# marcinjurek/pyMRA

Hardware: AMD Instinct MI355X
Metric: MRA nodes/sec, resident device pass (prior+posterior+likelihood+predict with tree and data in HBM; value_end_to_end = the same nodes over the wall-clock of MRATree(...)+getLikelihood()+predict()), 1024^2 grid M=6 J=4 r0=32 (higher is better)
Workload: dtype f64

## Files before the change

### pymra_amd/csrc/mra_kernels.h

```cpp
#pragma once
#include <hip/hip_runtime.h>
#include <stdint.h>

typedef double d4 __attribute__((ext_vector_type(4)));
typedef double d2 __attribute__((ext_vector_type(2)));
typedef int i4 __attribute__((ext_vector_type(4)));

#define MRA_AS1 __attribute__((address_space(1)))
__device__ __forceinline__ double gld(const double* p) { return *(const double MRA_AS1*)p; }
__device__ __forceinline__ int gldi(const int* p) { return *(const int MRA_AS1*)p; }
__device__ __forceinline__ d2 gld2(const double* p) { return *(const d2 MRA_AS1*)p; }
__device__ __forceinline__ d4 gld4(const double* p) { return *(const d4 MRA_AS1*)p; }
__device__ __forceinline__ void gst(double* p, double v) { *(double MRA_AS1*)p = v; }
__device__ __forceinline__ void gst2(double* p, d2 v) { *(d2 MRA_AS1*)p = v; }
__device__ __forceinline__ void gst4(double* p, d4 v) { *(d4 MRA_AS1*)p = v; }


#define MRA_YB 16
#ifdef MRA_WHATIF
#define MRA_WHATIF_BIT(dbg, bit) ((dbg) & (bit))
#else
#define MRA_WHATIF_BIT(dbg, bit) false
#endif
#define FT_LD 18
// ... 1841 lines not shown


#ifdef MRA_STAMPS
#define MRA_TSTAMP(slot) do { if (srow && (threadIdx.x & 63) == 0) srow[slot] = __builtin_amdgcn_s_memtime(); } while (0)
#define MRA_TSTAMP_ARG , unsigned long long* stamps
#define MRA_TSTAMP_ROW_ARG , unsigned long long* srow
#define MRA_TSTAMP_ROW(prob, t) , (stamps ? stamps + ((long)(prob) * 64 + (t)) * 8 : (unsigned long long*)nullptr)
#else
#define MRA_TSTAMP(slot) do { } while (0)
#define MRA_TSTAMP_ARG
#define MRA_TSTAMP_ROW_ARG
#define MRA_TSTAMP_ROW(prob, t)
#endif

__device__ __forceinline__ const double* trsm2_image_src(const Trsm2Prob& pb, int ntri, int e) {
    const int tile = e >> 7, chunk = e & 127, row = chunk >> 3, c2 = (chunk & 7) << 1;
    if (tile < ntri) {
        int jb = 1;
        while ((jb + 1) * jb / 2 <= tile) ++jb;
        const int kb = tile - jb * (jb - 1) / 2;
        return pb.L + (long)(jb * 16 + row) * pb.ldL + kb * 16 + c2;
    }
    return pb.invd + (long)(tile - ntri) * 256 + row * 16 + c2;
}

template <int I> struct Trsm2Step { static constexpr int value = I; };
template <int I, int N, class F>
__device__ __forceinline__ void trsm2_steps(int n, F f) {
    if constexpr (I < N) {
        if (I == 0 || I < n) { f(Trsm2Step<I>()); trsm2_steps<I + 1, N>(n, f); }
    }
}

template <int NTMAX, bool GATHER>
__device__ __forceinline__ void trsm2_row_tile(const Trsm2Prob& pb, const double* __restrict__ img, const int* __restrict__ sidx, int nt, int ntri,
                                               int t, int r, int q, int prow MRA_TSTAMP_ROW_ARG) {
    const d4 zero = {0, 0, 0, 0};
    MRA_TSTAMP(2);
    double* xp = pb.X + (long)t * 16 * pb.ldx + (long)r * pb.ldx + 4 * q;
    const double* lp = (pb.src && t >= pb.gtiles) ? pb.src + ((long)(t - pb.gtiles) * 16 + r) * pb.ldsrc + 4 * q : xp;
    d4 x[NTMAX];
    double ssq = 0.0;
    const bool with_var = pb.var && t >= pb.var_tile0;
    double* const vp = pb.var + (long)(t - pb.var_tile0) * 16 + r;
    if (nt <= 0) {
        if (with_var && q == 0) gst(vp, gld(vp) + pb.var_sign * ssq);
        return;
    }
    double var0 = 0.0;
    if (with_var && q == 0) var0 = gld(vp);
    if (GATHER) {
        const double* gp = pb.gW + t * 16 + r;
        trsm2_steps<0, NTMAX>(nt, [&](auto JB) __attribute__((always_inline)) {
            constexpr int jb = decltype(JB)::value;
            const i4 gi = *(const i4*)(sidx + jb * 16 + 4 * q);
#pragma unroll
            for (int j = 0; j < 4; ++j) x[jb][j] = gld(gp + (long)max(gi[j], 0) * pb.gld);
        });
    } else {
        trsm2_steps<0, NTMAX>(nt, [&](auto JB) __attribute__((always_inline)) { constexpr int jb = decltype(JB)::value; x[jb] = gld4(lp + jb * 16); });
    }
    if (GATHER) {
        trsm2_steps<0, NTMAX>(nt, [&](auto JB) __attribute__((always_inline)) {
            constexpr int jb = decltype(JB)::value;
            const i4 gi = *(const i4*)(sidx + jb * 16 + 4 * q);
#pragma unroll
            for (int j = 0; j < 4; ++j) x[jb][j] = gi[j] < 0 ? 0.0 : x[jb][j];
        });
    }
#ifdef MRA_STAMPS
    if (srow) { __builtin_amdgcn_s_waitcnt(0); MRA_TSTAMP(3); }
#endif
    trsm2_steps<0, NTMAX>(nt, [&](auto JB) __attribute__((always_inline)) {
        constexpr int jb = decltype(JB)::value;
        d4 acc = x[jb];
        d4 upd0 = zero, upd1 = zero;
#pragma unroll
        for (int kb = 0; kb < jb; ++kb) {
            const d4 a = *(const d4*)(img + (jb * (jb - 1) / 2 + kb) * 256 + prow * 16 + 4 * q);
            upd0 = mfma16(a[0], x[kb][0], upd0);
            upd1 = mfma16(a[1], x[kb][1], upd1);
            upd0 = mfma16(a[2], x[kb][2], upd0);
            upd1 = mfma16(a[3], x[kb][3], upd1);
        }
        if (jb > 0) acc -= upd0 + upd1;
        const d4 ia = *(const d4*)(img + (ntri + jb) * 256 + prow * 16 + 4 * q);
        d4 xx0 = mfma16(ia[0], acc[0], zero), xx1 = mfma16(ia[1], acc[1], zero);
        xx0 = mfma16(ia[2], acc[2], xx0);
        xx1 = mfma16(ia[3], acc[3], xx1);
        const d4 xx = xx0 + xx1;
        x[jb] = xx;
        gst4(xp + jb * 16, xx);
        ssq += xx[0] * xx[0] + xx[1] * xx[1] + xx[2] * xx[2] + xx[3] * xx[3];
    });
    MRA_TSTAMP(4);
    if (with_var) {
        ssq += __shfl_xor(ssq, 16, 64);
        ssq += __shfl_xor(ssq, 32, 64);
        if (q == 0) gst(vp, var0 + pb.var_sign * ssq);
    }
    MRA_TSTAMP(5);
}

template <int NTMAX>
__global__ __launch_bounds__(512) void k_trsm_rows2(const Trsm2Prob* __restrict__ probs, int tiles_per_wg MRA_TSTAMP_ARG) {
    extern __shared__ __attribute__((aligned(16))) double lds[];
    const Trsm2Prob pb = probs[blockIdx.y];
#ifdef MRA_STAMPS
    const unsigned long long t_wg0 = __builtin_amdgcn_s_memtime();
    const unsigned long long t_real0 = __builtin_amdgcn_s_memrealtime();
#endif
    const int t_begin = blockIdx.x * tiles_per_wg;
    if (t_begin >= pb.ntiles) return;
    const int t_end = min(pb.ntiles, t_begin + tiles_per_wg);
    const int nt = pb.nt;
    const int ntri = nt * (nt - 1) / 2;
    stage_chunks<8>(lds, (ntri + nt) * 128, [&](int e) -> const double* { return trsm2_image_src(pb, ntri, e); });
    int* const sidx = (int*)(lds + (long)(ntri + nt) * 256);
    if (pb.gtiles > 0 && t_begin < pb.gtiles)
        for (int e = threadIdx.x; e < nt * 16; e += blockDim.x) sidx[e] = gldi(pb.gidx + e);
    __syncthreads();
    const int wave = __builtin_amdgcn_readfirstlane(threadIdx.x >> 6), lane = threadIdx.x & 63, r = lane & 15, q = lane >> 4;
    const int nwave = blockDim.x >> 6;
    const int prow = pi16(r);
#ifdef MRA_STAMPS
    const unsigned long long t_wg1 = __builtin_amdgcn_s_memtime();
#endif
#ifdef MRA_STAMPS
#define MRA_T2_STAMP_HEAD(t) do { if (stamps && lane == 0) { stamps[((long)blockIdx.y * 64 + (t)) * 8 + 0] = t_wg0; stamps[((long)blockIdx.y * 64 + (t)) * 8 + 1] = t_wg1; } } while (0)
#define MRA_T2_STAMP_TAIL(t) do { if (stamps && lane == 0) { stamps[((long)blockIdx.y * 64 + (t)) * 8 + 6] = t_real0; stamps[((long)blockIdx.y * 64 + (t)) * 8 + 7] = __builtin_amdgcn_s_memrealtime(); } } while (0)
#else
#define MRA_T2_STAMP_HEAD(t) do { } while (0)
#define MRA_T2_STAMP_TAIL(t) do { } while (0)
#endif
    int t = t_begin + wave;
    for (; t < min(t_end, pb.gtiles); t += nwave) {
        MRA_T2_STAMP_HEAD(t);
        trsm2_row_tile<NTMAX, true>(pb, lds, sidx, nt, ntri, t, r, q, prow MRA_TSTAMP_ROW(blockIdx.y, t));
        MRA_T2_STAMP_TAIL(t);
    }
    for (; t < t_end; t += nwave) {
        MRA_T2_STAMP_HEAD(t);
        trsm2_row_tile<NTMAX, false>(pb, lds, sidx, nt, ntri, t, r, q, prow MRA_TSTAMP_ROW(blockIdx.y, t));
        MRA_T2_STAMP_TAIL(t);
    }
#undef MRA_T2_STAMP_HEAD
#undef MRA_T2_STAMP_TAIL
}

struct LeafSolveProb {
    const double* L;
    const double* invd;
    const double* V;
    const double* Ut;
    double* Wr;
    double* var;
    long ldL, ldx, ldw;
    int nt;
    int nrt;
    int nat;
    int zt;
};

#ifdef MRA_STAMPS
#define MRA_LSTAMP(slot) do { if (stamps && threadIdx.x == 0) stamps[(long)blockIdx.x * 8 + (slot)] = __builtin_amdgcn_s_memrealtime(); } while (0)
#define MRA_LSTAMP_ARG , unsigned long long* stamps
#else
#define MRA_LSTAMP(slot) do { } while (0)
#define MRA_LSTAMP_ARG
#endif
template <int NTMAX, int CT, bool LLDS>
__global__ __launch_bounds__(LLDS ? 512 : 256, LLDS ? 1 : 2) void k_leaf_solve_update(const LeafSolveProb* __restrict__ probs MRA_LSTAMP_ARG) {
    extern __shared__ __attribute__((aligned(16))) double lds[];
    MRA_LSTAMP(0);
    constexpr int NTHR = LLDS ? 512 : 256;
    constexpr int NWAVE = NTHR / 64;
    constexpr int NST = (CT * 64 + NTHR - 1) / NTHR;
    const LeafSolveProb* __restrict__ pp = probs + blockIdx.x;
    const int wave = __builtin_amdgcn_readfirstlane(threadIdx.x >> 6);
    const int lane = threadIdx.x & 63, r = lane & 15, q = lane >> 4;
// ... 2199 lines not shown
```

### pymra_amd/csrc/mra_plan.hip

```cpp
#include "mra_plan_types.h"
#include "mra_topology.h"
#include <atomic>
#include <chrono>
#include <memory>
#include <mutex>
#include <thread>

namespace {
struct PlanTrace {
    bool on;
    double t0, last;
    const char* what;
    static double now() { return std::chrono::duration<double, std::milli>(std::chrono::steady_clock::now().time_since_epoch()).count(); }
    explicit PlanTrace(const char* w) : on(getenv("MRA_TRACE_PLAN") != nullptr), t0(now()), last(t0), what(w) {}
    void mark(const char* label) { if (on) { const double t = now(); fprintf(stderr, "  [%s] %-34s %7.2f ms\n", what, label, t - last); last = t; } }
    ~PlanTrace() { if (on) fprintf(stderr, "  [%s] total %.2f ms (descriptor uploads of this thread so far: %ld, %.2f ms)\n", what, now() - t0, upload_stats().n, upload_stats().ms); }
};
}

#include <map>
#include <unordered_map>
namespace {
struct DevPool {
    std::mutex mu;
// ... 1099 lines not shown
    pl->gLeafSolve.upload(sp);
    pl->gLeafUpdatePlain.upload(in_order(d.upd, order));
    std::vector<LeafSolveProb> half;
    pl->hLeafSolveHalfPos.clear();
    for (size_t k = 0; k < n_small; ++k) {
        const LeafSolveProb& q = sp[k];
        const int h0 = (q.nrt + 1) / 2;
        for (int part = 0; part < 2; ++part) {
            LeafSolveProb h = q;
            const int t0 = part ? h0 : 0, t1 = part ? q.nrt : h0;
            if (t1 <= t0) continue;
            h.V = q.V + (size_t)t0 * 16 * q.ldx; h.Wr = q.Wr + (size_t)t0 * 16 * q.ldw; h.var = q.var + (size_t)t0 * 16; h.nrt = t1 - t0;
            half.push_back(h);
            pl->hLeafSolveHalfPos.push_back(k);
        }
    }
    pl->n_leaf_solve_half = half.size();
    pl->gLeafSolveHalf.upload(half);
    pl->hLeafSolve = sp; pl->hLeafSolveHalf = half;
    std::vector<long> lr0(nl);
    std::vector<unsigned char> lup(nl, 0);
    for (size_t t = 0; t < nl; ++t) lr0[t] = pl->row0[pl->leaf_nodes[t]];
    for (size_t k = 0; k < n_small; ++k) lup[order[k]] = 1;
    pl->leaf_row0_dev.upload(lr0); pl->leaf_upd_dev.upload(lup);
    const int nts = pl->trsm_small_nt;
    pl->leaf_solve_lds = (size_t)((nts * (nts - 1) / 2 + nts) * FT_SZ + 2 * nat_max * 16 * LG_LD) * sizeof(double);
    pl->leaf_solve_ok = n_small > 0 && nat_max <= 13 && nat_max > 0 && pl->leaf_solve_lds <= 160 * 1024 && pl->leaf_max_rows >= 128;
}

static void build_big_leaf_tiles(mra_plan* pl, const std::vector<size_t>& order, size_t n_small) {
    typedef mra_plan::PriorKeep K;
    if (pl->keep.dirty == K::Dirty::Oversized && !pl->stale.n_wg) pl->stale.swap(pl->big);
    pl->big.n_wg = pl->big.n_tiles = 0;
    if (!pl->regular || n_small >= order.size()) return;
    const size_t nl = pl->leaf_nodes.size();
    std::vector<long> first(nl + 1, 0);
    for (size_t t = 0; t < nl; ++t) first[t + 1] = first[t] + (pl->row1[pl->leaf_nodes[t]] - pl->row0[pl->leaf_nodes[t]]) / 16;
    const long per_wg = pl->cascade_stage_all ? 8 : pl->cascade_wpw;
    std::vector<long> wg0;
    std::vector<int> wgn;
    for (size_t k = n_small; k < order.size(); ++k) {
        const size_t t = order[k];
        for (long a = first[t]; a < first[t + 1]; a += per_wg) { wg0.push_back(a); wgn.push_back((int)std::min(per_wg, first[t + 1] - a)); }
        pl->big.n_tiles += first[t + 1] - first[t];
    }
    pl->big.n_wg = (long)wg0.size();
    pl->big.wg0.upload(wg0); pl->big.wgn.upload(wgn);
}

static void build_leaf(mra_plan* pl, const double* y) {
    PlanTrace tr("build_leaf");
    ArenaScope arena(&pl->arena);
    pl->cphantom_valid = false;
    pl->resid_lists = pl->resid_refused = false;
    pl->slv.valid = false; pl->slv.built = false;
    pl->cov.built = false;
    pl->sit.built = false;
    LeafDescs d;
    build_obs_lists(pl, y, d);
    tr.mark("observation lists");
    pl->panel.alloc(std::max<long>(pl->leaf_poff.back(), 1));
    pl->leafInv.alloc(std::max<long>(pl->leaf_ioff.back(), 1));
    tr.mark("panel allocation");
    build_leaf_descriptors(pl, d);
    tr.mark("leaf descriptors (host)");
    upload_leaf_ut_and_clear_panels(pl);
    tr.mark("panel memset");
    pl->hLeafSyrk = d.syrk;
    build_parent_products(pl, d);
    tr.mark("parent / grandparent descriptors");
    std::vector<size_t> order;
    const size_t n_small = order_small_first(pl, order);
    pl->n_chol_small = pl->n_trsm_small = n_small;
    upload_leaf_descriptors(pl, d, order);
    build_big_panels(pl, d);
    build_leaf_row_solves(pl, d, order, n_small);
    build_leaf_solve_lists(pl, d, order, n_small);
    build_big_leaf_tiles(pl, order, n_small);
    arena.finish();
    tr.mark("descriptor arena to the device");
// ... 23 lines not shown

template <int EPI>
static void launch_gemm(mra_plan* pl, const GemmProb* probs, size_t nprob, long maxM, long maxN, bool allow_lds = true, bool lower_tri = false) {
    mra_launch_gemm(pl, EPI, probs, nprob, maxM, maxN, allow_lds, lower_tri);
}
template <int EPI>
static void launch_leaf_gemm(mra_plan* pl, const GemmProb* probs, size_t nprob) { mra_launch_leaf_gemm(pl, EPI, probs, nprob); }

static void launch_panel(mra_plan* pl, const PanelProb* probs, size_t nprob, int accumulate = 0) {
    if (!nprob) return;
    hipLaunchKernelGGL(k_panel_chol, dim3((unsigned)nprob), dim3(256), 0, pl->stream, probs, pl->dnode.p, pl->errflag.p, accumulate);
}
void mra_panel_chol(mra_plan* pl, const PanelProb* probs, size_t nprob, double* dn, int* err) {
    hipLaunchKernelGGL(k_panel_chol, dim3((unsigned)nprob), dim3(256), 0, pl->stream, probs, dn, err, 0);
}
void mra_sample_draw(mra_plan* pl, const SampleZ& zs, long Kn, double* zc) {
    hipLaunchKernelGGL(k_sample_draw, dim3((unsigned)((Kn * 16 + 255) / 256)), dim3(256), 0, pl->stream, zs, Kn, zc);
}

#ifdef MRA_STAMPS
static unsigned long long* stamp_buffer(DevVec<double>& b, size_t n) {
    if (b.n < n) { b.alloc(n); HIP_TRY(mraMemset(b.p, 0, b.n * sizeof(double))); HIP_TRY(hipDeviceSynchronize()); }
    return (unsigned long long*)b.p;
}
#define MRA_TSTAMP_VAL , tst
#define MRA_LSTAMP_VAL , (unsigned long long*)pl->kstamps2.p
#define MRA_LSTAMP_NUL , (unsigned long long*)nullptr
#else
#define MRA_TSTAMP_VAL
#define MRA_LSTAMP_VAL
#define MRA_LSTAMP_NUL
#endif

static bool launch_trsm2(mra_plan* pl, const Trsm2Prob* probs, size_t nprob, int nt, long max_tiles, int tiles_per_wg) {
    if (!pl->prepare_only && (!nprob || max_tiles <= 0 || nt <= 0)) return true;
    if (nt > TRSM2_MAX_NT) return false;
    ensure_big_lds(pl, {(const void*)k_trsm_rows2<2>, (const void*)k_trsm_rows2<4>, (const void*)k_trsm_rows2<LEAF_SMALL_TILES>, (const void*)k_trsm_rows2<TRSM2_MAX_NT>});
    if (pl->prepare_only) return true;
    const size_t lds = (size_t)(nt * (nt - 1) / 2 + nt) * 2048 + (size_t)nt * 16 * sizeof(int);
    const unsigned gx = (unsigned)((max_tiles + tiles_per_wg - 1) / tiles_per_wg);
    const unsigned tb = 512;
#ifdef MRA_STAMPS
    unsigned long long* tst = (nprob >= 1024 && max_tiles <= 64) ? stamp_buffer(pl->tstamps, nprob * 64 * 8) : nullptr;
#endif
    for (size_t off = 0; off < nprob; off += 65535) {
        dim3 grid(gx, (unsigned)std::min<size_t>(65535, nprob - off));
        if (nt <= 2) hipLaunchKernelGGL((k_trsm_rows2<2>), grid, dim3(tb), lds, pl->stream, probs + off, tiles_per_wg MRA_TSTAMP_VAL);
        else if (nt <= 4) hipLaunchKernelGGL((k_trsm_rows2<4>), grid, dim3(tb), lds, pl->stream, probs + off, tiles_per_wg MRA_TSTAMP_VAL);
        else if (nt <= LEAF_SMALL_TILES) hipLaunchKernelGGL((k_trsm_rows2<LEAF_SMALL_TILES>), grid, dim3(tb), lds, pl->stream, probs + off, tiles_per_wg MRA_TSTAMP_VAL);
        else hipLaunchKernelGGL((k_trsm_rows2<TRSM2_MAX_NT>), grid, dim3(tb), lds, pl->stream, probs + off, tiles_per_wg MRA_TSTAMP_VAL);
    }
    return true;
}

static void launch_level_row_solve(mra_plan* pl, int m, const Trsm2Prob* probs2, const TrsmNode* nodes, double* var) {
    LevelData& lv = pl->lev[m];
    if (launch_trsm2(pl, probs2, lv.nodes.size(), lv.cwt, lv.max_tiles, 32)) return;
    ensure_tile_lists(pl, m);
    hipLaunchKernelGGL(k_trsm_rows, dim3((unsigned)((lv.ntiles + 3) / 4)), dim3(256), 0, pl->stream, nodes, lv.tile_node.p, lv.tile_row0.p,
                       lv.ntiles, pl->W.p, (long)pl->ldw, lv.c0, var);
}

static void launch_parent_front(mra_plan* pl, int nacc, size_t nprob, size_t lds, const FrontProb* probs, bool pair = false) {
    ensure_big_lds(pl, {(const void*)k_parent_front<2>, (const void*)k_parent_front<4>, (const void*)k_parent_front<8>, (const void*)k_parent_front<12>,
                        (const void*)k_parent_front_pair<17>, (const void*)k_parent_front_pair<23>});
    const dim3 grid((unsigned)nprob);
    if (pair) {
        if (nacc == 17) hipLaunchKernelGGL(k_parent_front_pair<17>, grid, dim3(256), lds, pl->stream, probs, pl->parentSegs.p, pl->dnode.p, pl->errflag.p);
        else hipLaunchKernelGGL(k_parent_front_pair<23>, grid, dim3(256), lds, pl->stream, probs, pl->parentSegs.p, pl->dnode.p, pl->errflag.p);
        return;
    }
    switch (nacc) {
        case 2: hipLaunchKernelGGL(k_parent_front<2>, grid, dim3(512), lds, pl->stream, probs, pl->parentSegs.p, pl->dnode.p, pl->errflag.p); break;
        case 4: hipLaunchKernelGGL(k_parent_front<4>, grid, dim3(512), lds, pl->stream, probs, pl->parentSegs.p, pl->dnode.p, pl->errflag.p); break;
        case 8: hipLaunchKernelGGL(k_parent_front<8>, grid, dim3(512), lds, pl->stream, probs, pl->parentSegs.p, pl->dnode.p, pl->errflag.p); break;
        default: hipLaunchKernelGGL(k_parent_front<12>, grid, dim3(512), lds, pl->stream, probs, pl->parentSegs.p, pl->dnode.p, pl->errflag.p); break;
    }
}

enum class LeafPart { All, Small, Rest };
// ... 197 lines not shown
    std::vector<PanelProb> ch = pl->hLeafCholSorted;
    std::vector<Trsm2Prob> ts = pl->hLeafTrsmFullPlainG;
    std::vector<LeafSolveProb> sp = pl->hLeafSolve, half = pl->hLeafSolveHalf;
    for (size_t k = 0; k < nl; ++k) {
        const size_t t = order[k];
        ch[k].src = C0(t); ch[k].obs = pl->obs_idx.p + pl->obs_off_host[t]; ch[k].n_obs = pl->leaf_nobs_host[t];
        ts[k].src = V0(t); ts[k].ldsrc = pl->leaf_nop[t];
        sp[k].V = V0(t);
    }
    for (size_t h = 0; h < half.size(); ++h) {
        const size_t k = pl->hLeafSolveHalfPos[h];
        half[h].V = sp[k].V + (half[h].V - pl->hLeafSolve[k].V);
    }
    pl->kLeafCholSorted.upload(ch); pl->kLeafTrsmFullPlainG.upload(ts);
    pl->kLeafSolve.upload(sp); pl->kLeafSolveHalf.upload(half);
    pl->resid_lists = true;
}

enum class PriorRows { RunAll, KeepAll, KeepRerunDirty };
struct PriorStep { bool run_knots = true; PriorRows rows = PriorRows::RunAll; };
static PriorStep prior_step_for(const mra_plan* pl, const PassRoute& r) {
    typedef mra_plan::PriorKeep K;
    PriorStep s;
    const K& k = pl->keep;
    if (r.path != PassPath::Fused || pl->host_cov || !pl->use_prior_reuse || (pl->dbg & 7) || !k.knots_valid) return s;
    s.run_knots = false;
    if (r.scatter_ut) return s;
    const bool have = (k.rows == K::Rows::All && k.var_valid) || (r.lik_rows && k.rows == K::Rows::Observed && k.dirty == K::Dirty::Clean);
    if (!have || k.dirty == K::Dirty::All) return s;
    s.rows = k.dirty == K::Dirty::Clean ? PriorRows::KeepAll : PriorRows::KeepRerunDirty;
    return s;
}

static CascadeArgs prior_cascade_base(const mra_plan* pl) {
    CascadeArgs base{};
    base.ycol = -1;
    for (int m = 0; m < pl->NL; ++m) {
        base.lev[m].kx = pl->fl[m].kx.p; base.lev[m].kvalid = pl->fl[m].kvalid.p; base.lev[m].Wk = pl->fl[m].Wk.p;
        base.lev[m].L = pl->lev[m].Lp.p; base.lev[m].invd = pl->lev[m].invP.p;
        base.coff[m] = pl->coff[m];
    }
    base.X = pl->X.p; base.W = pl->W.p; base.ldw = pl->ldw;
    return base;
}

static void run_prior_fused_knots(mra_plan* pl, const CascadeArgs& base) {
    const int n_chain = pl->route.n_chain;
    if (n_chain) {
        Work fl;
        for (int m = 0; m < n_chain; ++m) fl += pl->lev[m].fl_pchol;
        KTimer kt(pl, KF_PRIOR_CHOL, fl);
        KnotChainArgs ka{};
        for (int m = 0; m < n_chain; ++m) {
            ka.lev[m] = base.lev[m];
            ka.node_base[m] = (int)pl->level_ptr[m];
        }
        ka.chain = pl->kc_chain.p; ka.ownmask = pl->kc_ownmask.p; ka.knots = pl->kc_knots.p; ka.nl = n_chain; ka.err = pl->errflag.p;
#ifdef MRA_STAMPS
        ka.stamps = stamp_buffer(pl->kstamps, pl->lev[n_chain - 1].nodes.size() * 64);
#endif
        launch_knot_chain(pl, ka);
    }
    for (int m = n_chain; m < pl->NL; ++m) {
        LevelData& lv = pl->lev[m];
        KTimer kt(pl, KF_PRIOR_CHOL, lv.fl_pchol);
        CascadeArgs ar = base;
// ... 17 lines not shown
        fl.alg *= share; fl.exec *= share; fl.bytes = share * 8.0 * pl->P * (pl->d + 1 + pl->ldw + 1);
    }
    else if (r.lik_rows) {
        ensure_lik_tiles(pl);
        const double share = 16.0 * (double)pl->n_lik_tiles / (double)std::max<long>(pl->P, 1);
        fl.alg *= share; fl.exec *= share; fl.bytes = share * 8.0 * pl->P * (pl->d + 1 + pl->ldw) + pl->by_leaf_ut;
    }
    KTimer kt(pl, KF_PRIOR_TRSM, fl);
    CascadeArgs ar = base;
    ar.knot_mode = 0; ar.mlast = pl->NL - 1; ar.dbg = pl->dbg;
#ifdef MRA_STAMPS
    ar.stamps = stamp_buffer(pl->stamps, (size_t)pl->n_ftiles * 16);
#endif
    ar.var_out = pl->var.p; ar.cov0 = kernel_cov0(pl);
    ar.ycol = pl->Ka; ar.y = pl->y.p;
    if (r.scatter_ut) {
        ar.obs_pos = pl->obs_pos.p; ar.tile_leaf = pl->ft_leaf.p; ar.leaf_ut = pl->leaf_ut.p; ar.leaf_nop = pl->leaf_nop_dev.p;
        ar.y = pl->y.p;
        for (int m = 0; m < pl->NL; ++m) ar.ut_off[m] = pl->coff[m] - pl->asuf[pl->NL];
        ar.ut_yrow = pl->Ka - pl->asuf[pl->NL];
    }
    if (pl->cascade_stage_all) { ar.n_wg = pl->n_fwg_leaf; ar.wg_tile0 = pl->ft_wg0_leaf.p; ar.wg_ntiles = pl->ft_wgn_leaf.p; }
    else { ar.n_wg = pl->n_fwg; ar.wg_tile0 = pl->ft_wg0.p; ar.wg_ntiles = pl->ft_wgn.p; }
    ar.tile_row0 = pl->ft_row0.p; ar.tile_chain = pl->ft_chain.p;
    if (r.lik_rows) ar.var_out = nullptr;
    if (only) { ar.n_wg = only->n_wg; ar.wg_tile0 = only->wg0.p; ar.wg_ntiles = only->wgn.p; }
    else if (r.lik_rows) {
        ar.row_gather = pl->obs_idx.p; ar.tile_chain = pl->lik_chain.p; ar.tile_leaf = pl->lik_leaf.p;
        ar.n_wg = pl->n_lik_wg; ar.wg_tile0 = pl->lik_wg0.p; ar.wg_ntiles = pl->lik_wgn.p;
    }
    launch_cascade_any(pl, ar);
}

static void run_prior_refresh(mra_plan* pl, bool with_var) {
    KTimer kt(pl, KF_MISC, Work(0.0, 0.0, 8.0 * 16.0 * pl->n_ftiles * (MRA_YB + (with_var ? 3 : 1))));
    const long n = pl->n_ftiles * 64;
    if (n <= 0) return;
    hipLaunchKernelGGL(k_refresh_yblock, dim3((unsigned)((n + 255) / 256)), dim3(256), 0, pl->stream, pl->W.p, (long)pl->ldw, pl->Ka, pl->y.p,
                       pl->ft_row0.p, pl->n_ftiles, with_var ? pl->var.p : (double*)nullptr, pl->var_prior.p);
}

static void keep_prior_var(mra_plan* pl) {
    if (pl->var_prior.n != (size_t)pl->P) pl->var_prior.alloc((size_t)pl->P);
    KTimer kt(pl, KF_MISC, Work(0.0, 0.0, 16.0 * pl->P));
    HIP_TRY(hipMemcpyAsync(pl->var_prior.p, pl->var.p, (size_t)pl->P * sizeof(double), hipMemcpyDeviceToDevice, pl->stream));
}

static void run_prior_fused(mra_plan* pl) {
    typedef mra_plan::PriorKeep K;
    const PassRoute& r = pl->route;
    const PriorStep step = prior_step_for(pl, r);
    const CascadeArgs base = prior_cascade_base(pl);
    K& k = pl->keep;
    if (step.run_knots) {
        prior_keep_reset(pl);
        run_prior_fused_knots(pl, base);
        k.knots_valid = true;
    }
    switch (step.rows) {
        case PriorRows::RunAll:
            run_prior_fused_rows(pl, base);
            k.rows = r.lik_rows ? K::Rows::Observed : K::Rows::All;
            k.dirty = K::Dirty::Clean;
            pl->stale.n_wg = pl->stale.n_tiles = 0;
            if (!r.lik_rows && pl->use_prior_reuse) { keep_prior_var(pl); k.var_valid = true; }
            return;
        case PriorRows::KeepRerunDirty:
            run_prior_refresh(pl, !r.lik_rows);
            run_prior_fused_rows(pl, base, pl->stale.n_wg ? &pl->stale : &pl->big);
            k.dirty = K::Dirty::Clean;
            pl->stale.n_wg = pl->stale.n_tiles = 0;
            return;
        case PriorRows::KeepAll:
            run_prior_refresh(pl, !r.lik_rows);
            return;
    }
}

static void run_predict_hi(mra_plan* pl) {
    const int NL = pl->NL, nlo = NL - 4;
    PredHiArgs hi{};
    Work fl_hi, fl_lo;
    for (int h = 0; h < 4; ++h) {
        const int m = nlo + h;
        hi.hi[h].F = pl->lev[m].F.p; hi.hi[h].invF = pl->lev[m].invF.p; hi.hi[h].nf = pl->lev[m].nf;
        hi.hi[h].ld = pl->lev[m].ldf; hi.hi[h].stride = (long)pl->lev[m].nf * pl->lev[m].ldf;
        hi.coff_hi[h] = pl->coff[m];
        fl_hi += pl->lev[m].fl_trsm + pl->lev[m].fl_update;
    }
    hi.W = pl->W.p; hi.var = pl->var.p; hi.ldw = pl->ldw;
    hi.col_low = pl->coff[nlo - 1]; hi.n_low = nlo * 4 + 1; hi.lev0 = nlo;
    hi.tile_row0 = pl->ft_row0.p; hi.tile_chain = pl->ft_chain.p; hi.wg_tile0 = pl->ft_wg0.p; hi.wg_ntiles = pl->ft_wgn.p;
    fl_hi.bytes = 8.0 * pl->P * (pl->ldw + (pl->ldw - pl->coff[nlo - 1]) + 2);
    const bool fold = pl->route.update == LeafUpdate::InPredictHi;
    if (fold) {
        hi.wg_leaf = pl->hi_wgleaf.p; hi.leaf_ut = pl->leaf_ut.p; hi.leaf_nop = pl->leaf_nop_dev.p; hi.leaf_row0 = pl->leaf_row0_dev.p; hi.na = pl->na[NL];
        fl_hi += Work(pl->fl_leaf_update.alg, pl->fl_leaf_update.exec, pl->by_leaf_tt + pl->by_leaf_ut);
    }
    PredArgs lo{};
    for (int m = 0; m < nlo; ++m) {
        lo.lev[m].F = pl->lev[m].F.p; lo.lev[m].invF = pl->lev[m].invF.p; lo.lev[m].nf = pl->lev[m].nf;
        lo.lev[m].ld = pl->lev[m].ldf; lo.lev[m].stride = (long)pl->lev[m].nf * pl->lev[m].ldf;
        lo.coff[m] = pl->coff[m];
        fl_lo += pl->lev[m].fl_trsm + pl->lev[m].fl_update;
    }
    lo.deep = lo.lev[nlo - 1];
    lo.W = pl->W.p; lo.mean = pl->mean.p; lo.var = pl->var.p; lo.ldw = pl->ldw; lo.ycol = pl->Ka;
    lo.tile_row0 = pl->ft_row0.p; lo.tile_chain = pl->ft_chain.p; lo.wg_tile0 = pl->hi_wg0_8.p; lo.wg_ntiles = pl->hi_wgn_8.p;
// ... 33 lines not shown
    if (ar.n_wg <= 0) return;
    launch_predict_any(pl, ar, lds);
}

static void phase_mark(mra_plan* pl, int k) { if (k == 0 || k == 5 || pl->ktiming) hipEventRecord(pl->ev[k], pl->stream); }

static void ensure_gt(mra_plan* pl) {
    if (pl->Gt.p || pl->leaf_goff.back() == 0) return;
    pl->Gt.alloc(pl->leaf_goff.back());
    for (size_t k = 0; k < pl->hKids.size(); ++k)
        if (pl->kid_leaf[k] >= 0) pl->hKids[k].G = pl->Gt.p + pl->leaf_goff[pl->kid_leaf[k]];
    pl->asmKids.upload(pl->hKids);
    for (size_t t = 0; t < pl->hLeafSyrk.size(); ++t) pl->hLeafSyrk[t].C = pl->Gt.p + pl->leaf_goff[t];
    pl->gLeafSyrk.upload(pl->hLeafSyrk);
}

static const PassRoute& open_pass(mra_plan* pl, uint32_t flags, bool full_rows) {
    if (g_dry) refuse_dry_run();
    if (!(pl->have_locs && pl->have_obs && pl->have_kernel))
        throw MraError(MRA_ERR_STATE, "mra_run needs set_locs, set_obs and set_kernel first");
    HIP_TRY(mraSetDevice(pl->device));
    if (pl->pass_open) {
        pl->cphantom_valid = false;
        prior_keep_reset(pl);
        if (pl->side_pending) HIP_TRY(hipStreamWaitEvent(pl->stream, pl->ev_join, 0));
        HIP_TRY(hipStreamSynchronize(pl->stream));
        HIP_TRY(hipStreamSynchronize(pl->stream2));
        HIP_TRY(hipMemsetAsync(pl->errflag.p, 0, sizeof(int), pl->stream));
        for (auto& e : pl->kev) { hipEventDestroy(e.second.first); hipEventDestroy(e.second.second); }
        pl->kev.clear();
    }
    pl->side_pending = false;
    pl->split_pending = false;
    pl->pass_open = true;
    pl->run_flags = flags;
    pl->slv.valid = false;
    for (int k = 0; k < KF_COUNT; ++k) pl->kstat[k] = mra_plan::KStat();
    if (!pl->lik_general_valid && route_for(pl, flags, full_rows).lik_general) ensure_lik_general(pl);
    pl->route = route_for(pl, flags, full_rows);
    pl->route_set = true;
    const PassRoute& r = pl->route;
    pl->leaf_fork = pl->use_leaf_fork && r.path == PassPath::Fused && r.chol == LeafChol::TilesSplit &&
                    0 < pl->n_trsm_small && pl->n_trsm_small < pl->leaf_nodes.size();
    return pl->route;
}

static void run_init_yblock(mra_plan* pl, const PassRoute& r) {
    KTimer kt(pl, KF_MISC, 0);
    const long n = pl->P * MRA_YB;
    hipLaunchKernelGGL(k_init_yblock, dim3((unsigned)((n + 255) / 256)), dim3(256), 0, pl->stream, pl->W.p,
                       (long)pl->ldw, pl->Ka, pl->y.p, pl->P, r.acc_var ? pl->var.p : (double*)nullptr, pl->host_cov ? 0.0 : kernel_cov0(pl),
                       pl->host_cov ? pl->covdiag.p : (const double*)nullptr);
}

static void run_prior_level_one_launch(mra_plan* pl, const PassRoute& r, LevelData& lv) {
    const size_t nn = lv.nodes.size();
    { KTimer kt(pl, KF_PRIOR_CHOL, lv.fl_knot_resid); launch_gemm<EPI_COV>(pl, lv.gKnotResid.p, nn, lv.cw, lv.cw); }
    { KTimer kt(pl, KF_PRIOR_CHOL, lv.fl_pchol); launch_panel(pl, lv.gPriorChol.p, nn); }
    if (r.lik_general) {
        Work w = lv.fl_resid + lv.fl_trsm.with_bytes(0.0);
        w.alg *= lv.lik_share; w.exec *= lv.lik_share; w.bytes *= lv.lik_share;
        KTimer kt(pl, KF_PRIOR_RESID, w);
        mra_launch_prior_level(pl, lv.gResidLik.p, lv.gResidLik.n);
    } else {
        KTimer kt(pl, KF_PRIOR_RESID, lv.fl_resid + lv.fl_trsm.with_bytes(0.0));
        mra_launch_prior_level(pl, lv.gResidFused.p, lv.gResidFused.n);
// ... 70 lines not shown
static void run_leaf_noise(mra_plan* pl, const PassRoute& r, size_t nl) {
    if (!pl->noise_on || resid_out_of_place(pl, r)) return;
    KTimer kt(pl, KF_MISC, 0);
    hipLaunchKernelGGL(k_leaf_noise, dim3((unsigned)((nl + 3) / 4)), dim3(256), 0, pl->stream, pl->gLeaf.p, pl->leaf_nobs.p, pl->noise.p, (int)nl);
}

struct SideFork {
    mra_plan* pl; hipStream_t main_stream; bool side; hipEvent_t joined;
    SideFork(mra_plan* p, bool on, hipEvent_t after, hipEvent_t joined_) : pl(p), main_stream(p->stream), side(on), joined(joined_) {
        if (!side) return;
        if (after) {
            HIP_TRY(hipEventRecord(after, main_stream));
            HIP_TRY(hipStreamWaitEvent(pl->stream2, after, 0));
        }
        pl->stream = pl->stream2;
    }
    void join() {
        if (!side) return;
        pl->stream = main_stream;
        HIP_TRY(hipEventRecord(joined, pl->stream2));
    }
    ~SideFork() { pl->stream = main_stream; }
};

static void run_leaf_chol_and_solve(mra_plan* pl, const PassRoute& r, size_t nl) {
    const int obs_tiles = pl->leaf_max_nop / 16;
    const int row_tiles = r.predict ? pl->leaf_max_tiles_full : pl->leaf_max_tiles_lik;
    if (r.path != PassPath::Fused) { launch_leaf_chol(pl, r, nl); launch_trsm2(pl, r.trsm_all, nl, obs_tiles, row_tiles, row_tiles); return; }
    const size_t n_small = pl->n_trsm_small;
    const int small_row_tiles = (r.predict && !r.solve_fused) ? pl->trsm_small_tiles_full : pl->trsm_small_tiles_lik;
    const bool oop = resid_out_of_place(pl, r);
    auto kept = [&](const Trsm2Prob* p) { return (oop && p == pl->gLeafTrsmFullPlainG.p) ? pl->kLeafTrsmFullPlainG.p : p; };
    const Trsm2Prob *trsm_all = kept(r.trsm_all), *trsm_small = kept(r.trsm_small);
    auto solve_rest = [&] { launch_trsm2(pl, trsm_all + n_small, nl - n_small, obs_tiles, row_tiles, (nl - n_small) < 512 ? 4 : row_tiles); };
    if (pl->leaf_fork) {
        SideFork fork(pl, true, pl->ev_leaf_fork, pl->ev_leaf_join);
        launch_leaf_chol(pl, r, nl, LeafPart::Rest);
        solve_rest();
        fork.join();
    }
    launch_leaf_chol(pl, r, nl, pl->leaf_fork ? LeafPart::Small : LeafPart::All);
    if (n_small) launch_trsm2(pl, trsm_small, n_small, pl->trsm_small_nt, small_row_tiles, small_row_tiles);
    if (pl->leaf_fork) HIP_TRY(hipStreamWaitEvent(pl->stream, pl->ev_leaf_join, 0));
    else if (nl > n_small) solve_rest();
}

static void run_leaf_big_panels(mra_plan* pl, const PassRoute& r, size_t nl) {
    const int v = r.predict ? 0 : 1;
    for (size_t st = 0; st < pl->gBigPanel[v].size(); ++st) {
        launch_panel(pl, pl->gBigPanel[v][st].p, nl, st > 0 ? 1 : 0);
        if (pl->bigM[v][st] > 0 && pl->bigN[v][st] > 0)
            launch_gemm<EPI_SUB>(pl, pl->gBigTrail[v][st].p, nl, pl->bigM[v][st], pl->bigN[v][st]);
    }
}

static void run_leaf_factor(mra_plan* pl, const PassRoute& r, size_t nl) {
    KTimer kt(pl, KF_LEAF_CHOL, r.predict ? pl->fl_leaf_chol : pl->fl_leaf_chol_lik);
    if (r.chol != LeafChol::BigPanels) run_leaf_chol_and_solve(pl, r, nl);
    else run_leaf_big_panels(pl, r, nl);
}

static void run_leaf_syrk(mra_plan* pl, size_t nl) {
    ensure_gt(pl);
    KTimer kt(pl, KF_LEAF_SYRK, pl->fl_leaf_syrk);
    launch_gemm<EPI_SET>(pl, pl->gLeafSyrk.p, nl, pl->leaf_max_na, pl->leaf_max_na, false, true);
}

static void run_leaf_var(mra_plan* pl, const PassRoute& r) {
    if (r.var == LeafVar::None) return;
    KTimer kt(pl, KF_MISC, 0);
    ensure_row_leaf(pl);
    if (r.var == LeafVar::FinishVar)
        hipLaunchKernelGGL(k_leaf_finish_var, dim3((unsigned)((pl->P + 255) / 256)), dim3(256), 0, pl->stream, pl->row_leaf.p, pl->W.p,
                           (long)pl->ldw, pl->Ka, pl->var.p, pl->P);
    else
// ... 1666 lines not shown
```

### pymra_amd/csrc/mra_plan_types.h

```cpp
#pragma once
#include "mra_kernels.h"
#include "../../include/mra_hip.h"

#include <algorithm>
#include <cmath>
#include <cstdio>
#include <cstdlib>
#include <cstring>
#include <dlfcn.h>
#include <functional>
#include <initializer_list>
#include <rccl/rccl.h>
#include <set>
#include <string>
#include <thread>
#include <vector>
#include <time.h>

#define MRA_VERSION_STR "mra_hip 0.2 (gfx950)"

static const bool g_dry = []() { const char* e = getenv("MRA_HOST_DRYRUN"); return e && e[0] == '1'; }();
hipError_t mraMalloc(void** p, size_t n);
hipError_t mraFree(void* p);
static inline hipError_t mraMemcpy(void* d, const void* s_, size_t n, hipMemcpyKind k) { if (g_dry) { memcpy(d, s_, n); return hipSuccess; } return hipMemcpy(d, s_, n, k); }
// ... 351 lines not shown
    struct PriorKeep {
        enum class Rows { None, Observed, All };
        enum class Dirty { Clean, Oversized, All };
        bool knots_valid = false;
        Rows rows = Rows::None;
        bool var_valid = false;
        Dirty dirty = Dirty::Clean;
    } keep;
    struct ResidKeep {
        enum class Form { None, COnly, Full };
        Form resid = Form::None;
        bool phantom = false;
    } rkeep;
    bool use_resid_reuse = true;
    DevVec<double> resid;
    std::vector<long> leaf_koff;
    bool resid_lists = false, resid_refused = false;
    std::vector<int> obs_list_host;
    std::vector<PanelProb> hLeafCholSorted;
    std::vector<Trsm2Prob> hLeafTrsmFullPlainG;
    std::vector<LeafSolveProb> hLeafSolve, hLeafSolveHalf;
    std::vector<size_t> hLeafSolveHalfPos;
    std::vector<LeafProb> hLeaf;
    DevVec<GemmProb> kLeafResid, kLeafResidLik;
    DevVec<PanelProb> kLeafCholSorted;
    DevVec<Trsm2Prob> kLeafTrsmFullPlainG;
    DevVec<LeafSolveProb> kLeafSolve, kLeafSolveHalf;
    DevVec<LeafProb> kLeaf;
    bool use_prior_reuse = true;
    DevVec<double> var_prior;
    struct LeafTileWgs {
        DevVec<long> wg0;
        DevVec<int> wgn;
        long n_wg = 0, n_tiles = 0;
        void swap(LeafTileWgs& o) { wg0.swap(o.wg0); wgn.swap(o.wgn); std::swap(n_wg, o.n_wg); std::swap(n_tiles, o.n_tiles); }
    } big, stale;
    int use_hi_fold = 1;
    bool use_prior_level = true;
    bool parent_panel_lds_ok = false;
    bool grand_syrk_dma_ok = false;
    bool grand_syrk_blk_ok = false;
    int use_syrk_blk = 1;
    bool seg_gemm_lds = true;
    bool use_pred_update = true;
    DevVec<long> leaf_row0_dev;
    DevVec<unsigned char> leaf_upd_dev;
    size_t leaf_solve_lds = 0;
    int leaf_solve_mode = 2;
    size_t n_trsm_small = 0;
    int trsm_small_nt = 0, trsm_small_tiles_full = 0, trsm_small_tiles_lik = 0;
    DevVec<GemmProb> gParentSyrk;
    DevVec<GemmSeg> parentSegs;
    DevVec<FrontProb> gParentFront;
    int parent_front_nacc = 0;
    size_t parent_front_lds = 0;
    int parent_pair_nacc = 0;
    size_t parent_pair_lds = 0;
    double parent_pair_idle_exec = 0;
    int use_parent_pair = 1;
    bool parent_syrk = false;
    bool lowrank_parent = false;
    DevVec<GemmProb> gParentPanel, gGrandSyrk;
    DevVec<GemmSeg> grandSegs, parentSegsAo;
    DevVec<FrontProb> gParentOwn;
    DevVec<Trsm2Prob> gParentZt;
    size_t parent_own_lds = 0;
    Work fl_parent_panel, fl_grand_syrk;
    bool shape_regular = false;
    std::vector<AsmChild> hKids;
// ... 337 lines not shown
```

Before: 1.719 million.

## Skip full prior refresh on kept passes by gathering y in leaf TRSM

On kept-prior passes the full-tile y-block and variance refresh is replaced by targeted work. The leaf triangular solve now gathers observations directly from y for the last gathered tile, zeroing missing or non-finite values. It reads the prior variance through an offset into the saved copy instead of restoring it. Only the big-leaf and empty-leaf tiles get a y-block refresh, and that refresh can run on the forked side stream. This removes a full-grid memory pass per predict call, at the cost of more control-flow state and more kernel instantiations.

```diff
diff --git a/pymra_amd/csrc/mra_kernels.h b/pymra_amd/csrc/mra_kernels.h
--- a/pymra_amd/csrc/mra_kernels.h
+++ b/pymra_amd/csrc/mra_kernels.h
@@ -1897,9 +1897,11 @@
     }
 }
 
-template <int NTMAX, bool GATHER>
+enum { TRSM2_STREAM = 0, TRSM2_GATHER = 1, TRSM2_YTILE = 2 };
+template <int NTMAX, int SRC>
 __device__ __forceinline__ void trsm2_row_tile(const Trsm2Prob& pb, const double* __restrict__ img, const int* __restrict__ sidx, int nt, int ntri,
-                                               int t, int r, int q, int prow MRA_TSTAMP_ROW_ARG) {
+                                               int t, int r, int q, int prow, const double* __restrict__ gy, long var_rd_off MRA_TSTAMP_ROW_ARG) {
+    constexpr bool GATHER = SRC == TRSM2_GATHER;
     const d4 zero = {0, 0, 0, 0};
     MRA_TSTAMP(2);
     double* xp = pb.X + (long)t * 16 * pb.ldx + (long)r * pb.ldx + 4 * q;
@@ -1909,11 +1911,11 @@
     const bool with_var = pb.var && t >= pb.var_tile0;
     double* const vp = pb.var + (long)(t - pb.var_tile0) * 16 + r;
     if (nt <= 0) {
-        if (with_var && q == 0) gst(vp, gld(vp) + pb.var_sign * ssq);
+        if (with_var && q == 0) gst(vp, gld(vp + var_rd_off) + pb.var_sign * ssq);
         return;
     }
     double var0 = 0.0;
-    if (with_var && q == 0) var0 = gld(vp);
+    if (with_var && q == 0) var0 = gld(vp + var_rd_off);
     if (GATHER) {
         const double* gp = pb.gW + t * 16 + r;
         trsm2_steps<0, NTMAX>(nt, [&](auto JB) __attribute__((always_inline)) {
@@ -1921,6 +1923,23 @@
             const i4 gi = *(const i4*)(sidx + jb * 16 + 4 * q);
 #pragma unroll
             for (int j = 0; j < 4; ++j) x[jb][j] = gld(gp + (long)max(gi[j], 0) * pb.gld);
+        });
+    } else if (SRC == TRSM2_YTILE) {
+        if (r == 0) {
+            trsm2_steps<0, NTMAX>(nt, [&](auto JB) __attribute__((always_inline)) {
+                constexpr int jb = decltype(JB)::value;
+                const i4 gi = *(const i4*)(sidx + jb * 16 + 4 * q);
+#pragma unroll
+                for (int j = 0; j < 4; ++j) x[jb][j] = gld(gy + max(gi[j], 0));
+            });
+        } else {
+            trsm2_steps<0, NTMAX>(nt, [&](auto JB) __attribute__((always_inline)) { constexpr int jb = decltype(JB)::value; x[jb] = zero; });
+        }
+        trsm2_steps<0, NTMAX>(nt, [&](auto JB) __attribute__((always_inline)) {
+            constexpr int jb = decltype(JB)::value;
+            const i4 gi = *(const i4*)(sidx + jb * 16 + 4 * q);
+#pragma unroll
+            for (int j = 0; j < 4; ++j) x[jb][j] = (gi[j] < 0 || !isfinite(x[jb][j])) ? 0.0 : x[jb][j];
         });
     } else {
         trsm2_steps<0, NTMAX>(nt, [&](auto JB) __attribute__((always_inline)) { constexpr int jb = decltype(JB)::value; x[jb] = gld4(lp + jb * 16); });
@@ -1967,8 +1986,8 @@
     MRA_TSTAMP(5);
 }
 
-template <int NTMAX>
-__global__ __launch_bounds__(512) void k_trsm_rows2(const Trsm2Prob* __restrict__ probs, int tiles_per_wg MRA_TSTAMP_ARG) {
+template <int NTMAX, bool LEAF>
+__device__ __forceinline__ void trsm2_rows(const Trsm2Prob* __restrict__ probs, int tiles_per_wg, const double* __restrict__ gy, long var_rd_off MRA_TSTAMP_ARG) {
     extern __shared__ __attribute__((aligned(16))) double lds[];
     const Trsm2Prob pb = probs[blockIdx.y];
 #ifdef MRA_STAMPS
@@ -1999,18 +2018,38 @@
 #define MRA_T2_STAMP_TAIL(t) do { } while (0)
 #endif
     int t = t_begin + wave;
-    for (; t < min(t_end, pb.gtiles); t += nwave) {
+    for (; t < min(t_end, pb.gtiles - (LEAF ? 1 : 0)); t += nwave) {
         MRA_T2_STAMP_HEAD(t);
-        trsm2_row_tile<NTMAX, true>(pb, lds, sidx, nt, ntri, t, r, q, prow MRA_TSTAMP_ROW(blockIdx.y, t));
+        trsm2_row_tile<NTMAX, TRSM2_GATHER>(pb, lds, sidx, nt, ntri, t, r, q, prow, gy, var_rd_off MRA_TSTAMP_ROW(blockIdx.y, t));
         MRA_T2_STAMP_TAIL(t);
+    }
+    if constexpr (LEAF) {
+        for (; t < min(t_end, pb.gtiles); t += nwave) {
+            MRA_T2_STAMP_HEAD(t);
+            trsm2_row_tile<NTMAX, TRSM2_YTILE>(pb, lds, sidx, nt, ntri, t, r, q, prow, gy, var_rd_off MRA_TSTAMP_ROW(blockIdx.y, t));
+            MRA_T2_STAMP_TAIL(t);
+        }
     }
     for (; t < t_end; t += nwave) {
         MRA_T2_STAMP_HEAD(t);
-        trsm2_row_tile<NTMAX, false>(pb, lds, sidx, nt, ntri, t, r, q, prow MRA_TSTAMP_ROW(blockIdx.y, t));
+        trsm2_row_tile<NTMAX, TRSM2_STREAM>(pb, lds, sidx, nt, ntri, t, r, q, prow, gy, var_rd_off MRA_TSTAMP_ROW(blockIdx.y, t));
         MRA_T2_STAMP_TAIL(t);
     }
 #undef MRA_T2_STAMP_HEAD
 #undef MRA_T2_STAMP_TAIL
+}
+#ifdef MRA_STAMPS
+#define MRA_TSTAMP_PASS , stamps
+#else
+#define MRA_TSTAMP_PASS
+#endif
+template <int NTMAX>
+__global__ __launch_bounds__(512) void k_trsm_rows2(const Trsm2Prob* __restrict__ probs, int tiles_per_wg MRA_TSTAMP_ARG) {
+    trsm2_rows<NTMAX, false>(probs, tiles_per_wg, nullptr, 0 MRA_TSTAMP_PASS);
+}
+template <int NTMAX>
+__global__ __launch_bounds__(512) void k_trsm_leaf_rows(const Trsm2Prob* __restrict__ probs, int tiles_per_wg, const double* __restrict__ gy, long var_rd_off MRA_TSTAMP_ARG) {
+    trsm2_rows<NTMAX, true>(probs, tiles_per_wg, gy, var_rd_off MRA_TSTAMP_PASS);
 }
 
 struct LeafSolveProb {
diff --git a/pymra_amd/csrc/mra_plan.hip b/pymra_amd/csrc/mra_plan.hip
--- a/pymra_amd/csrc/mra_plan.hip
+++ b/pymra_amd/csrc/mra_plan.hip
@@ -1155,20 +1155,29 @@
     typedef mra_plan::PriorKeep K;
     if (pl->keep.dirty == K::Dirty::Oversized && !pl->stale.n_wg) pl->stale.swap(pl->big);
     pl->big.n_wg = pl->big.n_tiles = 0;
-    if (!pl->regular || n_small >= order.size()) return;
+    pl->empty.n_tiles = 0; pl->empty_yblock_ok = false;
+    if (!pl->regular) return;
     const size_t nl = pl->leaf_nodes.size();
     std::vector<long> first(nl + 1, 0);
     for (size_t t = 0; t < nl; ++t) first[t + 1] = first[t] + (pl->row1[pl->leaf_nodes[t]] - pl->row0[pl->leaf_nodes[t]]) / 16;
+    std::vector<long> erow0;
+    for (size_t t = 0; t < nl; ++t)
+        if (pl->leaf_nop[t] == 0)
+            for (long a = first[t]; a < first[t + 1]; ++a) erow0.push_back(pl->row0[pl->leaf_nodes[t]] + 16 * (a - first[t]));
+    pl->empty.n_tiles = (long)erow0.size();
+    pl->empty.row0.upload(erow0);
+    if (n_small >= order.size()) return;
     const long per_wg = pl->cascade_stage_all ? 8 : pl->cascade_wpw;
-    std::vector<long> wg0;
+    std::vector<long> wg0, row0;
     std::vector<int> wgn;
     for (size_t k = n_small; k < order.size(); ++k) {
         const size_t t = order[k];
         for (long a = first[t]; a < first[t + 1]; a += per_wg) { wg0.push_back(a); wgn.push_back((int)std::min(per_wg, first[t + 1] - a)); }
+        for (long a = first[t]; a < first[t + 1]; ++a) row0.push_back(pl->row0[pl->leaf_nodes[t]] + 16 * (a - first[t]));
         pl->big.n_tiles += first[t + 1] - first[t];
     }
     pl->big.n_wg = (long)wg0.size();
-    pl->big.wg0.upload(wg0); pl->big.wgn.upload(wgn);
+    pl->big.wg0.upload(wg0); pl->big.wgn.upload(wgn); pl->big.row0.upload(row0);
 }
 
 static void build_leaf(mra_plan* pl, const double* y) {
@@ -1258,10 +1267,11 @@
 #define MRA_LSTAMP_NUL
 #endif
 
-static bool launch_trsm2(mra_plan* pl, const Trsm2Prob* probs, size_t nprob, int nt, long max_tiles, int tiles_per_wg) {
+static bool launch_trsm2(mra_plan* pl, const Trsm2Prob* probs, size_t nprob, int nt, long max_tiles, int tiles_per_wg, const double* leaf_y = nullptr, long var_rd_off = 0) {
     if (!pl->prepare_only && (!nprob || max_tiles <= 0 || nt <= 0)) return true;
     if (nt > TRSM2_MAX_NT) return false;
-    ensure_big_lds(pl, {(const void*)k_trsm_rows2<2>, (const void*)k_trsm_rows2<4>, (const void*)k_trsm_rows2<LEAF_SMALL_TILES>, (const void*)k_trsm_rows2<TRSM2_MAX_NT>});
+    ensure_big_lds(pl, {(const void*)k_trsm_rows2<2>, (const void*)k_trsm_rows2<4>, (const void*)k_trsm_rows2<LEAF_SMALL_TILES>, (const void*)k_trsm_rows2<TRSM2_MAX_NT>,
+                        (const void*)k_trsm_leaf_rows<2>, (const void*)k_trsm_leaf_rows<4>, (const void*)k_trsm_leaf_rows<LEAF_SMALL_TILES>, (const void*)k_trsm_leaf_rows<TRSM2_MAX_NT>});
     if (pl->prepare_only) return true;
     const size_t lds = (size_t)(nt * (nt - 1) / 2 + nt) * 2048 + (size_t)nt * 16 * sizeof(int);
     const unsigned gx = (unsigned)((max_tiles + tiles_per_wg - 1) / tiles_per_wg);
@@ -1271,7 +1281,13 @@
 #endif
     for (size_t off = 0; off < nprob; off += 65535) {
         dim3 grid(gx, (unsigned)std::min<size_t>(65535, nprob - off));
-        if (nt <= 2) hipLaunchKernelGGL((k_trsm_rows2<2>), grid, dim3(tb), lds, pl->stream, probs + off, tiles_per_wg MRA_TSTAMP_VAL);
+        if (leaf_y) {
+            if (nt <= 2) hipLaunchKernelGGL((k_trsm_leaf_rows<2>), grid, dim3(tb), lds, pl->stream, probs + off, tiles_per_wg, leaf_y, var_rd_off MRA_TSTAMP_VAL);
+            else if (nt <= 4) hipLaunchKernelGGL((k_trsm_leaf_rows<4>), grid, dim3(tb), lds, pl->stream, probs + off, tiles_per_wg, leaf_y, var_rd_off MRA_TSTAMP_VAL);
+            else if (nt <= LEAF_SMALL_TILES) hipLaunchKernelGGL((k_trsm_leaf_rows<LEAF_SMALL_TILES>), grid, dim3(tb), lds, pl->stream, probs + off, tiles_per_wg, leaf_y, var_rd_off MRA_TSTAMP_VAL);
+            else hipLaunchKernelGGL((k_trsm_leaf_rows<TRSM2_MAX_NT>), grid, dim3(tb), lds, pl->stream, probs + off, tiles_per_wg, leaf_y, var_rd_off MRA_TSTAMP_VAL);
+        }
+        else if (nt <= 2) hipLaunchKernelGGL((k_trsm_rows2<2>), grid, dim3(tb), lds, pl->stream, probs + off, tiles_per_wg MRA_TSTAMP_VAL);
         else if (nt <= 4) hipLaunchKernelGGL((k_trsm_rows2<4>), grid, dim3(tb), lds, pl->stream, probs + off, tiles_per_wg MRA_TSTAMP_VAL);
         else if (nt <= LEAF_SMALL_TILES) hipLaunchKernelGGL((k_trsm_rows2<LEAF_SMALL_TILES>), grid, dim3(tb), lds, pl->stream, probs + off, tiles_per_wg MRA_TSTAMP_VAL);
         else hipLaunchKernelGGL((k_trsm_rows2<TRSM2_MAX_NT>), grid, dim3(tb), lds, pl->stream, probs + off, tiles_per_wg MRA_TSTAMP_VAL);
@@ -1535,6 +1551,25 @@
     return s;
 }
 
+static bool kept_pass_needs_refresh(const mra_plan* pl, const PassRoute& r) {
+    if (r.lik_rows) return false;
+    if (!r.predict || r.update != LeafUpdate::InCascade || r.var != LeafVar::None || !pl->ut_gather) return true;
+    return pl->n_trsm_small > 0 && pl->trsm_small_nt == 0;
+}
+
+struct PriorHeadStep { bool rerun = false, yblock = false, yempty = false, side = false; };
+static PriorHeadStep prior_head_for(const mra_plan* pl, const PassRoute& r, const PriorStep& step) {
+    PriorHeadStep h;
+    if (step.rows == PriorRows::RunAll) return h;
+    h.rerun = step.rows == PriorRows::KeepRerunDirty;
+    if (kept_pass_needs_refresh(pl, r)) return h;
+    const bool rerun_big = h.rerun && pl->stale.n_wg == 0;
+    h.yblock = r.predict && pl->big.n_tiles > 0 && !rerun_big;
+    h.yempty = r.predict && pl->empty.n_tiles > 0 && !pl->empty_yblock_ok;
+    h.side = pl->leaf_fork && pl->stale.n_wg == 0 && resid_step_for(pl, r) == ResidStep::Keep;
+    return h;
+}
+
 static CascadeArgs prior_cascade_base(const mra_plan* pl) {
     CascadeArgs base{};
     base.ycol = -1;
@@ -1618,18 +1653,32 @@
     launch_cascade_any(pl, ar);
 }
 
-static void run_prior_refresh(mra_plan* pl, bool with_var) {
-    KTimer kt(pl, KF_MISC, Work(0.0, 0.0, 8.0 * 16.0 * pl->n_ftiles * (MRA_YB + (with_var ? 3 : 1))));
-    const long n = pl->n_ftiles * 64;
+static void run_prior_refresh(mra_plan* pl, bool with_var, const mra_plan::LeafTileWgs* only = nullptr) {
+    const long ntiles = only ? only->n_tiles : pl->n_ftiles;
+    KTimer kt(pl, KF_MISC, Work(0.0, 0.0, 8.0 * 16.0 * ntiles * (MRA_YB + (with_var ? 3 : 1))));
+    const long n = ntiles * 64;
     if (n <= 0) return;
     hipLaunchKernelGGL(k_refresh_yblock, dim3((unsigned)((n + 255) / 256)), dim3(256), 0, pl->stream, pl->W.p, (long)pl->ldw, pl->Ka, pl->y.p,
-                       pl->ft_row0.p, pl->n_ftiles, with_var ? pl->var.p : (double*)nullptr, pl->var_prior.p);
+                       only ? only->row0.p : pl->ft_row0.p, ntiles, with_var ? pl->var.p : (double*)nullptr, pl->var_prior.p);
 }
 
 static void keep_prior_var(mra_plan* pl) {
     if (pl->var_prior.n != (size_t)pl->P) pl->var_prior.alloc((size_t)pl->P);
     KTimer kt(pl, KF_MISC, Work(0.0, 0.0, 16.0 * pl->P));
     HIP_TRY(hipMemcpyAsync(pl->var_prior.p, pl->var.p, (size_t)pl->P * sizeof(double), hipMemcpyDeviceToDevice, pl->stream));
+}
+
+static void run_prior_rerun_dirty(mra_plan* pl, const CascadeArgs& base) {
+    run_prior_fused_rows(pl, base, pl->stale.n_wg ? &pl->stale : &pl->big);
+    pl->keep.dirty = mra_plan::PriorKeep::Dirty::Clean;
+    pl->stale.n_wg = pl->stale.n_tiles = 0;
+}
+
+static void run_prior_side_head(mra_plan* pl) {
+    const mra_plan::PriorHead h = pl->side_head;
+    pl->side_head = mra_plan::PriorHead::None;
+    if (h == mra_plan::PriorHead::Rerun) run_prior_rerun_dirty(pl, prior_cascade_base(pl));
+    else if (h == mra_plan::PriorHead::YBlock) run_prior_refresh(pl, false, &pl->big);
 }
 
 static void run_prior_fused(mra_plan* pl) {
@@ -1649,17 +1698,22 @@
             k.rows = r.lik_rows ? K::Rows::Observed : K::Rows::All;
             k.dirty = K::Dirty::Clean;
             pl->stale.n_wg = pl->stale.n_tiles = 0;
+            if (!r.lik_rows) pl->empty_yblock_ok = true;
             if (!r.lik_rows && pl->use_prior_reuse) { keep_prior_var(pl); k.var_valid = true; }
             return;
-        case PriorRows::KeepRerunDirty:
-            run_prior_refresh(pl, !r.lik_rows);
-            run_prior_fused_rows(pl, base, pl->stale.n_wg ? &pl->stale : &pl->big);
-            k.dirty = K::Dirty::Clean;
-            pl->stale.n_wg = pl->stale.n_tiles = 0;
+        case PriorRows::KeepRerunDirty: case PriorRows::KeepAll: {
+            const PriorHeadStep head = prior_head_for(pl, r, step);
+            if (kept_pass_needs_refresh(pl, r)) { run_prior_refresh(pl, !r.lik_rows); pl->empty_yblock_ok = true; }
+            else if (k.var_valid) pl->var_rd_off = pl->var_prior.p - pl->var.p;
+            if (head.yempty) { run_prior_refresh(pl, false, &pl->empty); pl->empty_yblock_ok = true; }
+            if (head.side) {
+                pl->side_head = head.rerun ? mra_plan::PriorHead::Rerun : head.yblock ? mra_plan::PriorHead::YBlock : mra_plan::PriorHead::None;
+                return;
+            }
+            if (head.rerun) run_prior_rerun_dirty(pl, base);
+            if (head.yblock) run_prior_refresh(pl, false, &pl->big);
             return;
-        case PriorRows::KeepAll:
-            run_prior_refresh(pl, !r.lik_rows);
-            return;
+        }
     }
 }
 
@@ -1759,6 +1813,8 @@
     }
     pl->side_pending = false;
     pl->split_pending = false;
+    pl->side_head = mra_plan::PriorHead::None;
+    pl->var_rd_off = 0;
     pl->pass_open = true;
     pl->run_flags = flags;
     pl->slv.valid = false;
@@ -1895,15 +1951,18 @@
     const bool oop = resid_out_of_place(pl, r);
     auto kept = [&](const Trsm2Prob* p) { return (oop && p == pl->gLeafTrsmFullPlainG.p) ? pl->kLeafTrsmFullPlainG.p : p; };
     const Trsm2Prob *trsm_all = kept(r.trsm_all), *trsm_small = kept(r.trsm_small);
-    auto solve_rest = [&] { launch_trsm2(pl, trsm_all + n_small, nl - n_small, obs_tiles, row_tiles, (nl - n_small) < 512 ? 4 : row_tiles); };
+    const double* const leaf_y = (pl->ut_gather && !r.scatter_ut) ? pl->y.p : nullptr;
+    const long vro = leaf_y ? pl->var_rd_off : 0;
+    auto solve_rest = [&] { launch_trsm2(pl, trsm_all + n_small, nl - n_small, obs_tiles, row_tiles, (nl - n_small) < 512 ? 4 : row_tiles, leaf_y, vro); };
     if (pl->leaf_fork) {
         SideFork fork(pl, true, pl->ev_leaf_fork, pl->ev_leaf_join);
+        run_prior_side_head(pl);
         launch_leaf_chol(pl, r, nl, LeafPart::Rest);
         solve_rest();
         fork.join();
     }
     launch_leaf_chol(pl, r, nl, pl->leaf_fork ? LeafPart::Small : LeafPart::All);
-    if (n_small) launch_trsm2(pl, trsm_small, n_small, pl->trsm_small_nt, small_row_tiles, small_row_tiles);
+    if (n_small) launch_trsm2(pl, trsm_small, n_small, pl->trsm_small_nt, small_row_tiles, small_row_tiles, leaf_y, vro);
     if (pl->leaf_fork) HIP_TRY(hipStreamWaitEvent(pl->stream, pl->ev_leaf_join, 0));
     else if (nl > n_small) solve_rest();
 }
diff --git a/pymra_amd/csrc/mra_plan_types.h b/pymra_amd/csrc/mra_plan_types.h
--- a/pymra_amd/csrc/mra_plan_types.h
+++ b/pymra_amd/csrc/mra_plan_types.h
@@ -407,9 +407,15 @@
     struct LeafTileWgs {
         DevVec<long> wg0;
         DevVec<int> wgn;
+        DevVec<long> row0;
         long n_wg = 0, n_tiles = 0;
-        void swap(LeafTileWgs& o) { wg0.swap(o.wg0); wgn.swap(o.wgn); std::swap(n_wg, o.n_wg); std::swap(n_tiles, o.n_tiles); }
+        void swap(LeafTileWgs& o) { wg0.swap(o.wg0); wgn.swap(o.wgn); row0.swap(o.row0); std::swap(n_wg, o.n_wg); std::swap(n_tiles, o.n_tiles); }
     } big, stale;
+    LeafTileWgs empty;
+    bool empty_yblock_ok = false;
+    enum class PriorHead { None, Rerun, YBlock };
+    PriorHead side_head = PriorHead::None;
+    long var_rd_off = 0;
     int use_hi_fold = 1;
     bool use_prior_level = true;
     bool parent_panel_lds_ok = false;
```

Result: faster. 1.768 million, median of 6 (+2.9%).
